# KamilSJaron/smudgeplot

Measured on NVIDIA H100. Metric: k-mers/sec scanned (hetmers) at 1/2/4/8 H100; bit-exact .smu vs ref C, higher is better.
Workload: dtype u64

## Files before the change

### include/hetmers_b200.h

```cpp
#ifndef HETMERS_B200_H
#define HETMERS_B200_H

#include <stdint.h>

#ifdef __cplusplus
extern "C" {
#endif

#define HM_SMAX        1000
#define HM_FMAX         500
#define HM_PLOT_W      (HM_FMAX+1)
#define HM_PLOT_CELLS  ((HM_SMAX+1)*(HM_FMAX+1))
#define HM_MAX_KMER      64
#define HM_MAX_SHARDS    16
#define HM_FILTER_MIN_BITS 22
#define HM_FILTER_MAX_BITS 37

#define HM_OK            0
#define HM_EINVAL       -1
#define HM_ECUDA        -2
#define HM_ENOMEM       -3
#define HM_EIO          -4
#define HM_EFORMAT      -5
#define HM_EUNSUPPORTED -6
// ... 51 lines not shown
                       unsigned long long *d_count, const hm_shards *shards, void *stream);

#define HM_SYMM_MIN_KMER 2

typedef struct hm_symm_layout
  { int64_t bytes;
    int64_t off_header;
    int64_t off_bloom;
    int64_t seg_words;
    int64_t off_cand_key, off_cand_lo, off_cand_meta;
    int64_t cand_cap;
    int64_t range;
    int64_t off_runs, runs_cap;
    int32_t n_seg, pad;
  } hm_symm_layout;

typedef struct hm_symm_shards
  { int32_t  n_seg, self;
    int64_t  off[HM_MAX_SHARDS+1];
    uint64_t first_key[HM_MAX_SHARDS];
  } hm_symm_shards;

#define HM_SYMM_ASYMMETRIC 1
#define HM_SYMM_OVERFLOW   2

int  hm_symm_plan(int64_t n, int64_t range, int kmer, int n_seg, hm_symm_layout *out);
void hm_symm_seeds(uint64_t seed[2]);
int  hm_k_symm_fingerprint(const uint64_t *d_keys, const uint64_t *d_keys_lo, const uint16_t *d_cnt,
                           int64_t i0, int64_t i1, int kmer, const uint64_t seed[2],
                           uint64_t *d_acc, void *stream);
int  hm_k_symm_runscan(const uint64_t *d_keys, const uint64_t *d_keys_lo, const uint16_t *d_cnt, int64_t n,
                       const void *d_bucket, int bits, int idx64, int kmer, int64_t lo, int64_t hi,
                       void *d_work, const hm_symm_layout *layout, const hm_symm_shards *shards, void *stream);
int  hm_k_symm_runs(const uint64_t *d_keys, const uint64_t *d_keys_lo, const uint16_t *d_cnt, int64_t n,
                    const void *d_bucket, int bits, int idx64, int kmer, int64_t lo, int64_t hi,
                    void *d_work, const hm_symm_layout *layout, const hm_symm_shards *shards, void *stream);
int  hm_k_symm_resolve(const uint64_t *d_keys, const uint64_t *d_keys_lo, const uint16_t *d_cnt, int64_t n,
                       const void *d_bucket, int bits, int idx64, int kmer,
                       void *d_work, const hm_symm_layout *layout, const hm_symm_shards *shards,
                       unsigned long long *d_plot, void *stream);
int  hm_k_symm_extract(const uint64_t *d_keys, const uint64_t *d_keys_lo, const uint16_t *d_cnt, int64_t n,
                       const void *d_bucket, int bits, int idx64, int kmer,
                       void *d_work, const hm_symm_layout *layout, const hm_symm_shards *shards,
                       const uint16_t *d_pixmap, int64_t c0, int64_t c1, hm_pair_rec *d_out, int64_t cap,
                       unsigned long long *d_count, void *stream);
int  hm_symm_status(const void *d_work, const hm_symm_layout *layout, uint64_t *n_cand, uint64_t *status,
                    void *stream);
int  hm_symm_align_cut(const uint64_t *d_keys, int64_t n, int kmer, int64_t cut, int64_t *out);

int hm_dev_alloc(int64_t bytes, void **dptr);
int hm_dev_free(void *dptr);
int hm_ipc_export(void *dptr, unsigned char handle[64]);
int hm_ipc_open(const unsigned char handle[64], void **dptr);
int hm_ipc_close(void *dptr);
int hm_p2p_native_atomics(int dev_a, int dev_b);

int hm_k_min_count(const uint16_t *d_cnt, int64_t frst, int64_t last, int *d_min, void *stream);

int hm_k_find_keys(const uint64_t *d_keys, const uint64_t *d_keys_lo, int64_t n,
                   const void *d_bucket, int bits, int idx64,
                   const uint64_t *d_query, const uint64_t *d_query_lo, int64_t nq,
                   int64_t *d_pos, void *stream);

int hm_pick_bucket_bits(int64_t n);


// ... 211 lines not shown
```

### smudgeplot_b200/_lib.py

```python
from __future__ import annotations

import ctypes as C
import os

HERE = os.path.dirname(os.path.abspath(__file__))
LIB_PATH = os.environ.get("HETMERS_LIB") or os.path.join(HERE, "lib", "libhetmers_b200.so")
BIN_PATH = os.path.join(HERE, "bin", "hetmers")

SMAX, FMAX = 1000, 500
PLOT_W = FMAX + 1
PLOT_CELLS = (SMAX + 1) * (FMAX + 1)

ABI_SYMBOLS = [
    "hm_last_error", "hm_abi_version", "hm_device_count", "hm_device_info",
    "hm_k_unpack_records", "hm_k_build_bucket_index", "hm_k_pass1_degree", "hm_k_pass2_plot",
    "hm_k_min_count", "hm_k_find_keys", "hm_pick_bucket_bits", "hm_k_pass2_extract", "hm_scan_extract", "hm_pass2_scratch_bytes",
    "hm_k_build_filter", "hm_filter_words", "hm_pick_filter_bits",
    "hm_dev_alloc", "hm_dev_free", "hm_ipc_export", "hm_ipc_open", "hm_ipc_close", "hm_p2p_native_atomics",
    "hm_scan_create", "hm_prewarm", "hm_set_io_threads", "hm_scan_destroy", "hm_scan_examine", "hm_scan_condition", "hm_scan_run", "hm_hetmers_host",
    "hm_scan_run_path", "hm_scan_is_symmetric", "hm_symm_plan", "hm_symm_seeds", "hm_k_symm_fingerprint", "hm_k_symm_runscan", "hm_k_symm_runs", "hm_k_symm_resolve",
    "hm_k_symm_extract",
    "hm_symm_status", "hm_symm_align_cut",
    "hm_scan_download", "hm_set_device_budget", "hm_stream_plan", "hm_stream_plan_shards", "hm_scan_residency", "hm_table_open", "hm_table_close", "hm_table_view", "hm_write_smu",
    "hm_rank_scan_create", "hm_rank_scan_destroy", "hm_rank_scan_cuts", "hm_rank_scan_pass1", "hm_rank_scan_bloom",
    "hm_rank_scan_prepare", "hm_rank_scan_slices", "hm_rank_scan_route", "hm_rank_scan_answer", "hm_rank_scan_settle",
    "hm_rank_scan_result", "hm_rank_scan_residency",
    "hm_rank_scan_extract_prepare", "hm_rank_scan_extract_slices", "hm_rank_scan_extract_route",
    "hm_rank_scan_extract_settle", "hm_rank_scan_extract_result", "hm_sort_pair_records",
    "hm_condition_range_bytes", "hm_condition_plan", "hm_scan_condition_files",
    "hm_table_write_open", "hm_table_write_buckets", "hm_table_write_append", "hm_table_write_close",
    "hm_table_write_abort", "hm_table_write_place", "hm_table_write_at", "hm_table_write_seal",
    "hm_set_condition_gpus",
    "hm_k_cond_hist", "hm_k_shard_route_count", "hm_k_shard_route_scatter", "hm_k_shard_settle_bytes",
    "hm_k_shard_settle", "hm_shard_condition_bytes",
    "hm_k_shard_route_count_window", "hm_k_shard_route_scatter_window", "hm_k_cond_pack", "hm_rank_condition_bytes",
    "hm_rank_condition_cut",
    "hm_rank_scan_extract_records", "hm_k_pairs_hist", "hm_k_pairs_route_count", "hm_k_pairs_route_scatter",
    "hm_pairs_sort_scratch_bytes", "hm_k_pairs_sort", "hm_k_pairs_label_bounds", "hm_k_pairs_format", "hm_pairs_bytes",
    "hm_scan_write_pairs", "hm_scan_pairs_hist", "hm_pair_windows",
]


class HostTable(C.Structure):
    _fields_ = [("kmer", C.c_int32), ("ibyte", C.c_int32), ("nparts", C.c_int32), ("minval", C.c_int32),
                ("nels", C.c_int64), ("index", C.POINTER(C.c_int64)), ("part_nels", C.POINTER(C.c_int64)),
                ("part_rec", C.POINTER(C.c_void_p)), ("part_fd", C.POINTER(C.c_int32)),
                ("part_fd_off", C.POINTER(C.c_int64))]


MAX_SHARDS = 16


class Shards(C.Structure):
# ... 90 lines not shown
    if not os.path.exists(LIB_PATH):
        raise ImportError(f"{LIB_PATH} is missing: run `make lib` (or __graft_entry__.build()); "
                          "the hetmers path has no CPU / PyTorch fallback")
    L = C.CDLL(LIB_PATH)
    vp, i32, i64 = C.c_void_p, C.c_int, C.c_int64
    L.hm_last_error.restype = C.c_char_p
    L.hm_device_info.argtypes = [i32, C.c_char_p, i32, C.POINTER(i32), C.POINTER(i64)]
    L.hm_k_unpack_records.argtypes = [vp, i64, i64, vp, i32, i32, vp, vp, vp, vp]
    L.hm_k_build_bucket_index.argtypes = [vp, i64, i32, vp, i32, vp]
    L.hm_k_pass1_degree.argtypes = [vp, vp, vp, i64, vp, i32, i32, vp, i32, i32, i64, i64, vp, vp, C.POINTER(Shards), vp]
    L.hm_dev_alloc.argtypes = [i64, C.POINTER(vp)]
    L.hm_dev_free.argtypes = [vp]
    L.hm_ipc_export.argtypes = [vp, C.c_char_p]
    L.hm_ipc_open.argtypes = [C.c_char_p, C.POINTER(vp)]
    L.hm_ipc_close.argtypes = [vp]
    L.hm_p2p_native_atomics.argtypes = [i32, i32]
    L.hm_k_build_filter.argtypes = [vp, i64, i32, vp, vp]
    L.hm_filter_words.argtypes = [i32]
    L.hm_filter_words.restype = i64
    L.hm_pick_filter_bits.argtypes = [i64]
    L.hm_k_pass2_plot.argtypes = [vp, vp, vp, i32, i64, i64, vp, C.POINTER(Shards), vp]
    L.hm_k_pass2_extract.argtypes = [vp, vp, vp, vp, vp, i32, i64, i64, vp, vp, i64, vp, C.POINTER(Shards), vp]
    L.hm_k_min_count.argtypes = [vp, i64, i64, vp, vp]
    L.hm_k_find_keys.argtypes = [vp, vp, i64, vp, i32, i32, vp, vp, i64, vp, vp]
    L.hm_pick_bucket_bits.argtypes = [i64]
    L.hm_pass2_scratch_bytes.argtypes = [i64, i32]
    L.hm_pass2_scratch_bytes.restype = i64
    L.hm_symm_plan.argtypes = [i64, i64, i32, i32, C.POINTER(SymmLayout)]
    L.hm_symm_seeds.argtypes = [C.POINTER(C.c_uint64)]
    L.hm_symm_seeds.restype = None
    L.hm_k_symm_fingerprint.argtypes = [vp, vp, vp, i64, i64, i32, C.POINTER(C.c_uint64), vp, vp]
    L.hm_k_symm_runscan.argtypes = [vp, vp, vp, i64, vp, i32, i32, i32, i64, i64, vp, C.POINTER(SymmLayout),
                                    C.POINTER(SymmShards), vp]
    L.hm_k_symm_runs.argtypes = [vp, vp, vp, i64, vp, i32, i32, i32, i64, i64, vp, C.POINTER(SymmLayout),
                                 C.POINTER(SymmShards), vp]
    L.hm_k_symm_resolve.argtypes = [vp, vp, vp, i64, vp, i32, i32, i32, vp, C.POINTER(SymmLayout),
                                    C.POINTER(SymmShards), vp, vp]
    L.hm_k_symm_extract.argtypes = [vp, vp, vp, i64, vp, i32, i32, i32, vp, C.POINTER(SymmLayout),
                                    C.POINTER(SymmShards), vp, i64, i64, vp, i64, vp, vp]
    L.hm_symm_status.argtypes = [vp, C.POINTER(SymmLayout), C.POINTER(C.c_uint64), C.POINTER(C.c_uint64), vp]
    L.hm_symm_align_cut.argtypes = [vp, i64, i32, i64, C.POINTER(i64)]
    L.hm_scan_create.argtypes = [C.POINTER(HostTable), C.POINTER(i32), i32, C.POINTER(vp)]
    L.hm_scan_destroy.argtypes = [vp]
    L.hm_scan_destroy.restype = None
    L.hm_scan_examine.argtypes = [vp, i32, C.POINTER(i32), C.POINTER(i32)]
    L.hm_scan_condition.argtypes = [vp, i32, i32, i32, C.POINTER(i64)]
    L.hm_scan_run.argtypes = [vp, vp, C.POINTER(ScanStats)]
    L.hm_scan_run_path.argtypes = [vp, i32, vp, C.POINTER(ScanStats)]
    L.hm_scan_is_symmetric.argtypes = [vp]
    L.hm_scan_extract.argtypes = [vp, vp, C.POINTER(C.POINTER(PairRec)), C.POINTER(i64)]
    L.hm_hetmers_host.argtypes = [C.POINTER(HostTable), C.POINTER(i32), i32, vp, C.POINTER(ScanStats)]
    L.hm_scan_download.argtypes = [vp, vp, vp, vp, vp]
    L.hm_set_device_budget.argtypes = [i64]
    L.hm_set_device_budget.restype = None
    L.hm_stream_plan.argtypes = [i64, i32, i32, i64, C.POINTER(StreamLayout)]
    L.hm_stream_plan_shards.argtypes = [i64, i32, i32, i64, i32, C.POINTER(StreamLayout)]
    L.hm_scan_residency.argtypes = [vp, C.POINTER(i64), C.POINTER(i64)]
    u64p, i64p = C.POINTER(C.c_uint64), C.POINTER(i64)
    L.hm_rank_scan_create.argtypes = [C.POINTER(HostTable), i32, i32, i32, u64p, C.POINTER(vp)]
    L.hm_rank_scan_destroy.argtypes = [vp]
    L.hm_rank_scan_destroy.restype = None
    L.hm_rank_scan_cuts.argtypes = [vp, i64p, u64p]
    L.hm_rank_scan_pass1.argtypes = [vp, u64p]
    L.hm_rank_scan_bloom.argtypes = [vp, C.POINTER(vp), i64p]
    L.hm_rank_scan_prepare.argtypes = [vp, i32, i64p, i64p]
    L.hm_rank_scan_slices.argtypes = [vp, i64, i64p, C.POINTER(vp), C.POINTER(vp), C.POINTER(vp), C.POINTER(vp)]
# ... 68 lines not shown
```

### smudgeplot_b200/csrc/hm_symm.cu

```cuda
#include <cuda_runtime.h>
#include <stdint.h>
#include <stdio.h>
#include <stdlib.h>
#include <string.h>

#include "hetmers_b200.h"
#include "hm_internal.h"
#include "hm_device.cuh"

#define RS_THREADS 256
#define RS_EPT     8
#define RS_TILE    (RS_THREADS*RS_EPT)
#define RS_HALO    64
#define RS_WIN     (RS_TILE+2*RS_HALO)
#define RS_SCANCAP RS_HALO
#define RS_RUNCAP  (RS_HALO+1)
#define RS_LONGRUN 32
#ifndef RS_MINBLOCKS
#define RS_MINBLOCKS 6
#endif
#ifndef RS_STAGE
#define RS_STAGE   384
#endif

#define SY_STATUS_ASYMMETRIC 1ull
#define SY_STATUS_OVERFLOW   2ull

#define SY_HDR_CAND   0
#define SY_HDR_STATUS 1
#define SY_HDR_RUNS   2
#define SY_HDR_S      3
#define SY_HDR_PEND   4
#define SY_HDR_QUERY  5

struct SymmView
  { unsigned long long *cand_n;
    unsigned long long *status;
    uint32_t *bloom;
    uint32_t  seg_words;
    int       n_seg, self;
    uint64_t  first_key[HM_MAX_SHARDS];
    uint64_t *cand_key, *cand_lo, *cand_meta;
    unsigned long long cand_cap;
    unsigned long long *runs_n;
    uint64_t *runs;
    unsigned long long runs_cap;
    uint64_t *s_key, *s_lo;
    unsigned long long s_cap;
    const hm_stream_sview *sviews;
    uint64_t *pend, *pend_key, *pend_lo;
    uint64_t *q_key, *q_lo, *q_tag;
    unsigned long long pend_cap, q_cap;
  };

template <int KW>
__device__ __forceinline__ void bloom_slot(const SymmView &W, int seg, int kmer, uint64_t hi, uint64_t lo,
// ... 204 lines not shown
static int l2_persist(void)
{ const char *e = getenv("HETMERS_L2_PERSIST");
  return (e == NULL || strcmp(e,"0") != 0);
}

static SymmView make_view(void *d_work, const hm_symm_layout *L, const hm_symm_shards *sh)
{ SymmView W;
  uint8_t *b = (uint8_t *) d_work;
  memset(&W,0,sizeof(W));
  W.cand_n    = (unsigned long long *) (b + L->off_header) + SY_HDR_CAND;
  W.status    = W.cand_n + SY_HDR_STATUS;
  W.bloom     = (uint32_t *) (b + L->off_bloom);
  W.seg_words = (uint32_t) L->seg_words;
  W.n_seg     = L->n_seg;
  W.self      = 0;
  if (sh != NULL && sh->n_seg > 1)
    { W.self = sh->self;
      for (int r = 0; r < sh->n_seg; r++) W.first_key[r] = sh->first_key[r];
    }
  W.cand_key  = (uint64_t *) (b + L->off_cand_key);
  W.cand_lo   = (uint64_t *) (b + L->off_cand_lo);
  W.cand_meta = (uint64_t *) (b + L->off_cand_meta);
  W.cand_cap  = (unsigned long long) L->cand_cap;
  W.runs_n    = W.cand_n + SY_HDR_RUNS;
  W.runs      = (uint64_t *) (b + L->off_runs);
  W.runs_cap  = (unsigned long long) L->runs_cap;
  return W;
}


template <int KW> struct RsSmem
  { uint64_t *key, *klo;
    uint16_t *cnt;
    uint64_t *ckey, *clo, *cmeta;
    uint16_t *t1;
    uint16_t *t2r;
  };

__device__ __forceinline__ uint64_t pack_meta(int cx, int cy, int pos, int yb)
{ return (uint64_t) cx | ((uint64_t) cy << 16) | ((uint64_t) pos << 32) | ((uint64_t) yb << 40); }

#ifdef RS_PROBE
__device__ int rs_probe_mode;
#define RS_PROBE_IS(m) (rs_probe_mode == (m))
#else
#define RS_PROBE_IS(m) false
#endif

template <int KW>
__device__ __forceinline__ void stage_candidates(const RsSmem<KW> &S, unsigned *s_nc, const SymmView &W,
                                                 bool emit, uint64_t x, uint64_t xl, uint64_t meta,
                                                 int lane, unsigned lt)
{ const unsigned bal = __ballot_sync(0xffffffffu,emit);
  if (bal == 0 || RS_PROBE_IS(4))
    return;
  unsigned base = 0;
  if (lane == 0)
    base = atomicAdd(s_nc,(unsigned) __popc(bal));
  base = __shfl_sync(0xffffffffu,base,0);
  const unsigned at = base + __popc(bal & lt);
  const bool     over = emit && (at >= RS_STAGE);
  if (emit && !over)
    { S.ckey[at] = x;
      if (KW == 2) S.clo[at] = xl;
      S.cmeta[at] = meta;
    }
  if (base + __popc(bal) <= RS_STAGE)
    return;
  const unsigned ob = __ballot_sync(0xffffffffu,over);
  unsigned long long g0 = 0;
  if (lane == 0)
    g0 = atomicAdd(W.cand_n,(unsigned long long) __popc(ob));
  g0 = __shfl_sync(0xffffffffu,g0,0) + (unsigned long long) __popc(ob & lt);
  if (over)
    { if (g0 < W.cand_cap)
        { W.cand_key[g0] = x;
          if (KW == 2) W.cand_lo[g0] = xl;
          W.cand_meta[g0] = meta;
        }
      else
        atomicOr(W.status,SY_STATUS_OVERFLOW);
    }
}

template <int KW>
__device__ __forceinline__ void s_push(const SymmView &W, uint64_t x, uint64_t xl)
{ const unsigned m = __activemask();
  const int      lane = threadIdx.x & 31, lead = __ffs(m)-1;
  unsigned long long at = 0;
  if (lane == lead)
    at = atomicAdd(W.cand_n + SY_HDR_S,(unsigned long long) __popc(m));
  at = __shfl_sync(m,at,lead) + (unsigned long long) __popc(m & ((1u << lane)-1));
  if (at < W.s_cap)
    { W.s_key[at] = x;
      if (KW == 2) W.s_lo[at] = xl;
    }
  else
    atomicOr(W.status,SY_STATUS_OVERFLOW);
}

template <int KW, bool SL>
__device__ __forceinline__ void bloom_insert(const SymmView &W, int kmer, uint64_t x, uint64_t xl)
{ uint64_t *word, mask;
  bloom_slot<KW>(W,W.self,kmer,x,xl,word,mask);
  if (!RS_PROBE_IS(3) || mask == (uint64_t) (uintptr_t) word)
    red_or64(word,mask);
  if (SL)
    s_push<KW>(W,x,xl);
}

#define RS_FLUSH ((RS_STAGE+RS_THREADS-1)/RS_THREADS)
struct RsFlush { uint64_t key[RS_FLUSH], lo[RS_FLUSH], meta[RS_FLUSH]; };

template <int KW>
__device__ __forceinline__ void flush_reserve(const RsSmem<KW> &S, unsigned long long *s_cb,
                                              unsigned long long *s_rb, const SymmView &W,
                                              unsigned nc, unsigned nr, RsFlush &F)
{ if (threadIdx.x == 0)
    { if (nc > 0) *s_cb = atomicAdd(W.cand_n,(unsigned long long) nc);
      if (nr > 0) *s_rb = atomicAdd(W.runs_n,(unsigned long long) nr);
    }
#pragma unroll
  for (int j = 0; j < RS_FLUSH; j++)
    { const unsigned i = threadIdx.x + j*RS_THREADS;
      if (i < nc)
        { F.key[j] = S.ckey[i];
          if (KW == 2) F.lo[j] = S.clo[i];
          F.meta[j] = S.cmeta[i];
        }
    }
}

template <int KW>
__device__ __forceinline__ void flush_store(const RsSmem<KW> &S, unsigned long long cb, unsigned long long rb,
                                            const SymmView &W, unsigned nc, unsigned nr, int64_t T0,
                                            const RsFlush &F)
{
#pragma unroll
  for (int j = 0; j < RS_FLUSH; j++)
    { const unsigned i = threadIdx.x + j*RS_THREADS;
      if (i < nc)
        { if (cb+i < W.cand_cap)
            { W.cand_key[cb+i] = F.key[j];
              if (KW == 2) W.cand_lo[cb+i] = F.lo[j];
              W.cand_meta[cb+i] = F.meta[j];
            }
          else
            atomicOr(W.status,SY_STATUS_OVERFLOW);
        }
    }
  for (unsigned i = threadIdx.x; i < nr; i += RS_THREADS)
    if (rb+i < W.runs_cap)
      W.runs[rb+i] = (uint64_t) (T0 + ((int) S.t2r[i] - RS_HALO));
    else
      atomicOr(W.status,SY_STATUS_OVERFLOW);
}

template <typename IdxT, int KW, bool SL>
__global__ void __launch_bounds__(256)
runs_kernel(const uint64_t *__restrict__ keys, const uint64_t *__restrict__ keys_lo,
            const uint16_t *__restrict__ cnt, int64_t n, const IdxT *__restrict__ bucket, int bshift,
            int kmer, int64_t lo, int64_t hi, const SymmView W)
// ... 65 lines not shown
                          if (KW == 2) W.cand_lo[base] = xl;
                          W.cand_meta[base] = meta;
                        }
                      else
                        atomicOr(W.status,SY_STATUS_OVERFLOW);
                    }
                }
            }
        }
    }
}

template <int KW> struct RunSfx    { typedef uint64_t T; };
template <>       struct RunSfx<1> { typedef uint32_t T; };

template <int KW>
__device__ __forceinline__ typename RunSfx<KW>::T run_sfx(uint64_t hi, uint64_t lo, int Pr)
{ if constexpr (KW == 1)
    return (uint32_t) ((hi << 2*Pr) >> 32);
  else
    return (hi << (2*Pr-32) << 32) | (lo >> (64-2*Pr));
}

template <typename T>
__device__ __forceinline__ bool one_base_in_run(T d, int Pr, int &pos)
{ const T u = (d | (d >> 1)) & (T) HM_M5;
  if constexpr (sizeof(T) == 4) pos = Pr + (__clz((int) d) >> 1);
  else                          pos = Pr + (__clzll((long long) d) >> 1);
  return (u & (u-1)) == 0;
}

template <int KW, bool SL, int LMAX>
__device__ __forceinline__ bool settle_members(const RsSmem<KW> &S, const SymmView &W, int kmer, int Pr, int pup,
                                               int h, int L, int a, bool in, bool own, int lane,
                                               uint64_t &x, uint64_t &xl, uint64_t &meta)
{ int Hx = 0, Ux = 0, part = 0, ppos = 0, cx = 0;
  if (in)
    { x  = S.key[h+a];
      xl = KW == 2 ? S.klo[h+a] : 0;
      cx = S.cnt[h+a];
      auto mate = [&](int b)
        { int pos;
          if (b < L && b != a && one_base_in_run(run_sfx<KW>(x ^ S.key[h+b],KW == 2 ? xl ^ S.klo[h+b] : 0,Pr),Pr,pos) &&
              cx + (int) S.cnt[h+b] <= HM_SMAX)
            { Hx += 1;
              if (pos >= pup) Ux += 1;
              part = b; ppos = pos;
            }
        };
      if constexpr (LMAX > 0)
        {
#pragma unroll
          for (int b = 0; b < LMAX; b++)
            mate(b);
        }
      else
        for (int b = 0; b < L; b++)
          mate(b);
      if (own && Ux > 0)
        bloom_insert<KW,SL>(W,kmer,x,xl);
    }
  const int pl = lane + part - a;
  int       Hy = __shfl_sync(0xffffffffu,Hx,pl & 31);
  if (!in || !own || Hx != 1 || part < a)
    return false;
  const uint64_t y = S.key[h+part], yl = KW == 2 ? S.klo[h+part] : 0;
  const int      cy = S.cnt[h+part];
  if (pl > 31)
    { Hy = 0;
      for (int b = 0; b < L; b++)
        { int pos;
          if (b != part && one_base_in_run(run_sfx<KW>(y ^ S.key[h+b],KW == 2 ? yl ^ S.klo[h+b] : 0,Pr),Pr,pos) &&
              cy + (int) S.cnt[h+b] <= HM_SMAX)
            Hy += 1;
        }
    }
  if (Hy != 1)
    return false;
  meta = pack_meta(cx,cy,ppos,base_at<KW>(y,yl,ppos));
  return true;
}

#ifdef RS_PROBE
#define RS_PHASES 8
#define RS_COLS   (RS_PHASES+3)
#define RS_PROBE_SLOTS 1024
__device__ unsigned long long rs_probe_cycles[RS_PROBE_SLOTS*RS_COLS];
#define RS_PROBE_TILE(b)  (rs_probe_mode == 2 ? (b) % 64 : (b))
#define RS_PROBE_START    __shared__ long long rs_t0, rs_t1; \
                          long long rs_t = clock64(); unsigned long long rs_acc[RS_PHASES] = {0, 0, 0, 0, 0, 0, 0, 0}; \
                          if (threadIdx.x == 0) rs_t0 = rs_t;
#define RS_PROBE_MARK(ph) { const long long t_ = clock64(); rs_acc[ph] += (unsigned long long) (t_ - rs_t); rs_t = t_; }
#define RS_PROBE_LANDED() if (threadIdx.x == 0) rs_t1 = clock64();
#define RS_PROBE_ALLDONE  const long long rs_t2 = clock64();
#define RS_PROBE_ROW      (rs_probe_cycles + (blockIdx.x % RS_PROBE_SLOTS)*RS_COLS)
#define RS_PROBE_FLUSH()  { if (lane == 0) _Pragma("unroll") for (int p_ = 0; p_ < RS_PHASES; p_++) \
                              atomicAdd(RS_PROBE_ROW + p_,rs_acc[p_]); }
#define RS_PROBE_LIFE()   { const long long t3_ = clock64(); \
                            if (threadIdx.x == 0) { atomicAdd(RS_PROBE_ROW + RS_PHASES,  (unsigned long long) (rs_t1 - rs_t0)); \
                                             atomicAdd(RS_PROBE_ROW + RS_PHASES+1,(unsigned long long) (rs_t2 - rs_t1)); \
                                             atomicAdd(RS_PROBE_ROW + RS_PHASES+2,(unsigned long long) (t3_ - rs_t2)); } }
#define RS_PROBE_LOADONLY() if (rs_probe_mode == 1) { RS_PROBE_FLUSH(); return; }
#define RS_PROBE_NOTAIL()   if (rs_probe_mode == 6) { RS_PROBE_FLUSH(); return; }

extern "C" int hm_probe_runscan(int mode, unsigned long long *cycles)
{ static unsigned long long rows[RS_PROBE_SLOTS*RS_COLS];
  cudaError_t e = cudaDeviceSynchronize();
  if (e == cudaSuccess && cycles != NULL)
    { e = cudaMemcpyFromSymbol(rows,rs_probe_cycles,sizeof(rows));
      for (int p = 0; p < RS_COLS; p++)
        { cycles[p] = 0;
          for (int r = 0; r < RS_PROBE_SLOTS; r++)
            cycles[p] += rows[r*RS_COLS+p];
        }
    }
  memset(rows,0,sizeof(rows));
  if (e == cudaSuccess)
    e = cudaMemcpyToSymbol(rs_probe_cycles,rows,sizeof(rows));
  if (e == cudaSuccess)
    e = cudaMemcpyToSymbol(rs_probe_mode,&mode,sizeof(mode));
  return e == cudaSuccess ? HM_OK : hm_cuda_fail(e,"hm_probe_runscan");
}
#else
#define RS_PROBE_TILE(b)  (b)
#define RS_PROBE_START
#define RS_PROBE_MARK(ph)
#define RS_PROBE_LANDED()
#define RS_PROBE_ALLDONE
#define RS_PROBE_FLUSH()
#define RS_PROBE_LIFE()
#define RS_PROBE_LOADONLY()
#define RS_PROBE_NOTAIL()
#endif

template <typename IdxT, int KW, bool SL>
__global__ void __launch_bounds__(RS_THREADS,RS_MINBLOCKS)
runscan_kernel(const uint64_t *__restrict__ keys, const uint64_t *__restrict__ keys_lo,
               const uint16_t *__restrict__ cnt, int64_t n, const IdxT *__restrict__ bucket, int bshift,
               int kmer, int64_t lo, int64_t hi, int64_t tile0, int use_tma, const SymmView W)
{ extern __shared__ __align__(128) uint8_t smem[];
  __shared__ __align__(8) uint64_t s_bar;
  __shared__ unsigned s_nc, s_nr;
  __shared__ unsigned long long s_base[2];
  RsSmem<KW> S;
  S.key   = (uint64_t *) smem;
  S.klo   = S.key + (KW == 2 ? RS_WIN : 0);
  S.ckey  = S.key + KW*RS_WIN;
  S.clo   = S.ckey + (KW == 2 ? RS_STAGE : 0);
  S.cmeta = S.ckey + KW*RS_STAGE;
  S.cnt   = (uint16_t *) (S.cmeta + RS_STAGE);
  S.t1    = S.cnt + RS_WIN;
  S.t2r   = S.t1 + RS_TILE/2;

  const int      Pr   = kmer >> 1;
  const int      pup  = kmer - Pr;
  const int      psh  = 64-2*Pr;
  const uint64_t pmask = ~(uint64_t) 0 << psh;
  const unsigned FULL = 0xffffffffu;
  const int      lane = threadIdx.x & 31;
  const int      warp = threadIdx.x >> 5;
  const unsigned lt   = (1u << lane) - 1;
  RS_PROBE_START

  const int64_t T0 = (tile0 + RS_PROBE_TILE(blockIdx.x)) * RS_TILE;
  const int64_t ws = T0 - RS_HALO;
  const int64_t e0 = ws > 0 ? ws : 0;
  const int64_t e1 = T0+RS_TILE+RS_HALO < n ? T0+RS_TILE+RS_HALO : n;
  const int     v0 = (int) (e0-ws), v1 = (int) (e1-ws);

  const int m   = v1-v0;
  const int mt  = use_tma ? (m & ~7) : 0;
  if (threadIdx.x == 0)
    { s_nc = 0; s_nr = 0;
      if (mt > 0)
        { mbar_init(&s_bar,1);
          fence_proxy_async_smem();
        }
    }
  __syncthreads();
  if (threadIdx.x == 0 && mt > 0)
    { mbar_arrive_expect_tx(&s_bar,(unsigned) (mt*(8*KW+2)));
      bulk_copy_g2s(S.key+v0,keys+e0,(unsigned) (8*mt),&s_bar);
      if (KW == 2)
// ... 59 lines not shown
        if (s0+32 > a1)   act &= (a1-s0 <= 0)  ? 0u : (0xffffffffu >> (s0+32-a1));
        const unsigned more = (em1 & E) | (E & ep1) | (em1 & em2);
        m2 = (E & ~em1 & ~ep1) & act;
        m3 = more & act & ~em1;
      }
    const int c2 = __popc(m2), c3 = __popc(m3);
    int pre2 = c2, pre3 = c3;
#pragma unroll
    for (int o = 1; o <= RS_EPT; o <<= 1)
      { int v2 = __shfl_up_sync(FULL,pre2,o), v3 = __shfl_up_sync(FULL,pre3,o);
        if (lane >= o) { pre2 += v2; pre3 += v3; }
      }
    n1 = __shfl_sync(FULL,pre2,RS_EPT);
    n3 = __shfl_sync(FULL,pre3,RS_EPT);
    int at = pre2-c2;
    while (m2 != 0)
      { my1[at++] = (uint16_t) (wd*32 + __ffs(m2)-1);
        m2 &= m2-1;
      }
    at = n1 + pre3-c3;
    while (m3 != 0)
      { my1[at++] = (uint16_t) (wd*32 + __ffs(m3)-1);
        m3 &= m3-1;
      }
  }
  __syncwarp();
  if (RS_PROBE_IS(5))
    n3 = 0;
  RS_PROBE_MARK(2)

  for (int i0 = 0; i0 < n1; i0 += 32)
    { const int i = i0+lane;
      bool     emit = false;
      uint64_t x = 0, xl = 0, meta = 0;
      if (i < n1)
        { const int w = my1[i];
          x = S.key[w];
          const uint64_t y = S.key[w+1];
          uint64_t yl = 0;
          if (KW == 2) { xl = S.klo[w]; yl = S.klo[w+1]; }
          const int cx = S.cnt[w], cy = S.cnt[w+1];
          int pos;
          if (one_base_in_run(run_sfx<KW>(x ^ y,xl ^ yl,Pr),Pr,pos) && cx+cy <= HM_SMAX)
            { emit = true;
              meta = pack_meta(cx,cy,pos,base_at<KW>(y,yl,pos));
              if (pos >= pup)
                { bloom_insert<KW,SL>(W,kmer,x,xl);
                  bloom_insert<KW,SL>(W,kmer,y,yl);
                }
            }
        }
      stage_candidates<KW>(S,&s_nc,W,emit,x,xl,meta,lane,lt);
    }
  RS_PROBE_MARK(3)

  const int b1 = hi-T0 < RS_TILE+RS_HALO ? RS_HALO + (int) (hi-T0) : RS_WIN;
  for (int i0 = 0; i0 < n3; i0 += 32)
    { const int i = i0+lane;
      const int h = i < n3 ? my1[n1+i] : 0;
      int       L = 0;
      {
        const int      t  = (h >> 5) - (wd0-1);
        const unsigned w0 = __shfl_sync(FULL,eqw,t & 31), w1 = __shfl_sync(FULL,eqw,(t+1) & 31);
        const unsigned up = __funnelshift_r(w0,w1,h & 31);
        if (i < n3)
          L = (~up != 0) ? __ffs((int) ~up) : 33;
      }
      const int Ls = L <= 8 ? L : 0;
      int inc = Ls;
#pragma unroll
      for (int o = 1; o < 32; o <<= 1)
        { const int v = __shfl_up_sync(FULL,inc,o);
          if (lane >= o) inc += v;
        }
      const int M = __shfl_sync(FULL,inc,31);
      for (int t0 = 0; t0 < M; t0 += 32)
        { const int t = t0+lane;
          int r = 0;
#pragma unroll
          for (int s = 16; s > 0; s >>= 1)
            if (__shfl_sync(FULL,inc,r+s-1) <= t) r += s;
          const int hr = __shfl_sync(FULL,h,r), Lr = __shfl_sync(FULL,Ls,r);
          const int a  = t - (__shfl_sync(FULL,inc,r) - Lr);
          bool     emit = false;
          uint64_t x = 0, xl = 0, meta = 0;
          emit = settle_members<KW,SL,8>(S,W,kmer,Pr,pup,hr,Lr,a,t < M,hr+a < b1,lane,x,xl,meta);
          stage_candidates<KW>(S,&s_nc,W,emit,x,xl,meta,lane,lt);
        }
      unsigned lb = __ballot_sync(FULL,L > 8);
      while (lb != 0)
        { const int src = __ffs(lb)-1;
          lb &= lb-1;
          const int hh = __shfl_sync(FULL,h,src);
          int       LL = __shfl_sync(FULL,L,src);
          if (LL > 32)
            { const uint64_t xh = S.key[hh];
              while (LL <= RS_RUNCAP)
                { const int      t = hh+LL+lane;
                  const unsigned sb = __ballot_sync(FULL,t < RS_WIN && ((S.key[t] ^ xh) & pmask) == 0);
                  if (sb != FULL) { LL += __ffs(~sb)-1; break; }
                  LL += 32;
                }
            }
          if (LL > RS_RUNCAP || hh+LL >= RS_WIN)
            { if (lane == 0)
                S.t2r[atomicAdd(&s_nr,1u)] = (uint16_t) hh;
              continue;
            }
          for (int a0 = 0; a0 < LL; a0 += 32)
            { const int a = a0+lane;
              bool     emit = false;
              uint64_t x = 0, xl = 0, meta = 0;
              emit = settle_members<KW,SL,0>(S,W,kmer,Pr,pup,hh,LL,a,a < LL,hh+a < b1,lane,x,xl,meta);
              stage_candidates<KW>(S,&s_nc,W,emit,x,xl,meta,lane,lt);
            }
        }
    }
  RS_PROBE_MARK(4)
  RS_PROBE_NOTAIL()

  __syncthreads();
  RS_PROBE_MARK(5)
  RS_PROBE_ALLDONE
  if (RS_PROBE_IS(4))
    { RS_PROBE_FLUSH() return; }
  const unsigned nc = s_nc < RS_STAGE ? s_nc : RS_STAGE, nr = s_nr;
  if (nc == 0 && nr == 0)
    { RS_PROBE_MARK(6) RS_PROBE_LIFE() RS_PROBE_FLUSH() return; }
  RsFlush F;
  flush_reserve<KW>(S,&s_base[0],&s_base[1],W,nc,nr,F);
  __syncthreads();
  RS_PROBE_MARK(6)
  flush_store<KW>(S,s_base[0],s_base[1],W,nc,nr,T0,F);
  RS_PROBE_MARK(7)
  RS_PROBE_LIFE()
  RS_PROBE_FLUSH()
}

template <typename IdxT, int KW, bool SL>
__global__ void __launch_bounds__(RS_THREADS,RS_MINBLOCKS)
runscan_dense_kernel(const uint64_t *__restrict__ keys, const uint64_t *__restrict__ keys_lo,
                     const uint16_t *__restrict__ cnt, int64_t n, int kmer, int64_t lo, int64_t hi,
                     int64_t tile0, int use_tma, const SymmView W)
{ extern __shared__ __align__(128) uint8_t smem[];
  __shared__ __align__(8) uint64_t s_bar;
  __shared__ unsigned s_nc, s_nl;
  __shared__ unsigned long long s_base[2];
  __shared__ unsigned s_eq[RS_WIN/32+1];
  RsSmem<KW> S;
  S.key   = (uint64_t *) smem;
  S.klo   = S.key + (KW == 2 ? RS_WIN : 0);
  S.ckey  = S.key + KW*RS_WIN;
  S.clo   = S.ckey + (KW == 2 ? RS_STAGE : 0);
  S.cmeta = S.ckey + KW*RS_STAGE;
  S.cnt   = (uint16_t *) (S.cmeta + RS_STAGE);
  S.t1    = S.cnt + RS_WIN;
  S.t2r   = S.t1 + RS_WIN;
  uint16_t *s_part = S.t2r + RS_TILE/8;
  unsigned *hu = (unsigned *) (s_part + RS_WIN);
  uint32_t *rem = hu + RS_WIN/2;

  const int      Pr   = kmer >> 1, pup = kmer - Pr, psh = 64-2*Pr;
  const uint64_t pmask = ~(uint64_t) 0 << psh;
  const unsigned FULL = 0xffffffffu;
  const int      lane = threadIdx.x & 31;
  const int      warp = threadIdx.x >> 5;
  const unsigned lt   = (1u << lane) - 1;

  const int64_t T0 = (tile0 + blockIdx.x) * RS_TILE;
  const int64_t ws = T0 - RS_HALO;
  const int64_t e0 = ws > 0 ? ws : 0;
  const int64_t e1 = T0+RS_TILE+RS_HALO < n ? T0+RS_TILE+RS_HALO : n;
  const int     v0 = (int) (e0-ws), v1 = (int) (e1-ws);

  const int m   = v1-v0;
  const int mt  = use_tma ? (m & ~7) : 0;
  if (threadIdx.x == 0)
    { s_nc = 0; s_nl = 0;
      if (mt > 0)
        { mbar_init(&s_bar,1);
          fence_proxy_async_smem();
        }
    }
  for (int j = threadIdx.x; j < RS_WIN/2; j += RS_THREADS)
    hu[j] = 0;
  __syncthreads();
  if (threadIdx.x == 0 && mt > 0)
    { mbar_arrive_expect_tx(&s_bar,(unsigned) (mt*(8*KW+2)));
// ... 70 lines not shown
        { const uint32_t rx = rem[i];
          for (int j = i+1; j <= i+fwd; j++)
            { const uint32_t d = rx ^ rem[j];
              const uint32_t u = (d | (d>>1)) & 0x55555555u;
              if ((u & (u-1)) == 0 && cx + (int) S.cnt[j] <= HM_SMAX)
                { const int      pos = Pr + (__clz((int) d) >> 1);
                  const unsigned inc = 1u | (pos >= pup ? 0x100u : 0u);
                  atomicAdd(hu + (i>>1), inc << (16*(i&1)));
                  atomicAdd(hu + (j>>1), inc << (16*(j&1)));
                  s_part[i] = (uint16_t) j;
                  s_part[j] = (uint16_t) i;
                }
            }
        }
      else
        { const uint64_t x = S.key[i], xl = KW == 2 ? S.klo[i] : 0;
          for (int j = i+1; j <= i+fwd; j++)
            { int pos;
              if (one_base_apart<KW>(x,xl,S.key[j],KW == 2 ? S.klo[j] : 0,pos) && cx + (int) S.cnt[j] <= HM_SMAX)
                { const unsigned inc = 1u | (pos >= pup ? 0x100u : 0u);
                  atomicAdd(hu + (i>>1), inc << (16*(i&1)));
                  atomicAdd(hu + (j>>1), inc << (16*(j&1)));
                  s_part[i] = (uint16_t) j;
                  s_part[j] = (uint16_t) i;
                }
            }
        }
    }
  __syncthreads();

  for (int i0 = RS_HALO + (threadIdx.x & ~31); i0 < RS_HALO+RS_TILE; i0 += RS_THREADS)
    { const int i = i0+lane;
      bool     emit = false;
      uint64_t x = 0, xl = 0, meta = 0;
      if (i >= a0 && i < a1 && S.t1[i] != 0xffff)
        { const unsigned c = (hu[i>>1] >> (16*(i&1))) & 0xffffu;
          const int H = (int) (c & 0xff), U = (int) (c >> 8);
          if (H > 0)
            { x = S.key[i];
              if (KW == 2) xl = S.klo[i];
              if (U > 0)
                bloom_insert<KW,SL>(W,kmer,x,xl);
              const int j = s_part[i];
              if (H == 1 && j > i && ((hu[j>>1] >> (16*(j&1))) & 0xffu) == 1)
                { const uint64_t y = S.key[j], yl = KW == 2 ? S.klo[j] : 0;
                  int pos;
                  one_base_apart<KW>(x,xl,y,yl,pos);
                  emit = true;
                  meta = pack_meta(S.cnt[i],S.cnt[j],pos,base_at<KW>(y,yl,pos));
                }
            }
        }
      stage_candidates<KW>(S,&s_nc,W,emit,x,xl,meta,lane,lt);
    }

  __syncthreads();
  const unsigned nc = s_nc < RS_STAGE ? s_nc : RS_STAGE, nr = s_nl;
  if (nc == 0 && nr == 0)
    return;
  RsFlush F;
  flush_reserve<KW>(S,&s_base[0],&s_base[1],W,nc,nr,F);
  __syncthreads();
  flush_store<KW>(S,s_base[0],s_base[1],W,nc,nr,T0,F);
}

template <typename I, int K> struct Inst { typedef I IdxT; static constexpr int KW = K; };

template <class F>
static cudaError_t dispatch(int kmer, int idx64, F f)
{ if (kmer <= 32)
    return idx64 ? f(Inst<uint64_t,1>()) : f(Inst<uint32_t,1>());
  return idx64 ? f(Inst<uint64_t,2>()) : f(Inst<uint32_t,2>());
}

template <typename IdxT, int KW, bool SL = false>
static cudaError_t launch_runscan(const uint64_t *keys, const uint64_t *keys_lo, const uint16_t *cnt, int64_t n,
                                  const void *bucket, int bits, int kmer, int64_t lo, int64_t hi,
                                  const SymmView &W, cudaStream_t st)
{ static int configured[64] = {0};
  int dev = 0;
  cudaGetDevice(&dev);
  int64_t tile0 = lo/RS_TILE, tile1 = (hi+RS_TILE-1)/RS_TILE;
  int     tma   = ((((uintptr_t) keys) | ((uintptr_t) cnt) | ((uintptr_t) (keys_lo ? keys_lo : keys))) & 15) == 0;
  const int   Pr  = kmer >> 1;
  double      lam = (2*Pr >= 62) ? 0.0 : (double) n / (double) ((uint64_t) 1 << (2*Pr));
  bool        dense = (lam > 0.6);
  const char *force = getenv("HETMERS_RUNSCAN");
  if (force != NULL && strcmp(force,"dense") == 0)  dense = true;
  if (force != NULL && strcmp(force,"sparse") == 0) dense = false;
  cudaError_t e;
  if (dense)
    { size_t smem = (size_t) RS_WIN*(8*KW+2) + (size_t) RS_STAGE*8*(KW+1) +
                    2*(size_t) (RS_WIN+RS_TILE/8+RS_WIN) + 4*(size_t) (RS_WIN/2+RS_WIN);
      if (smem > 48*1024 && (dev >= 64 || !(configured[dev] & 2)))
        { e = cudaFuncSetAttribute(runscan_dense_kernel<IdxT,KW,SL>,cudaFuncAttributeMaxDynamicSharedMemorySize,(int) smem);
          if (e != cudaSuccess) return e;
          if (dev < 64) configured[dev] |= 2;
        }
      runscan_dense_kernel<IdxT,KW,SL><<<(unsigned) (tile1-tile0),RS_THREADS,smem,st>>>
          (keys,keys_lo,cnt,n,kmer,lo,hi,tile0,tma,W);
    }
  else
    { size_t smem = (size_t) RS_WIN*(8*KW+2) + (size_t) RS_STAGE*8*(KW+1) +
                    2*(size_t) (RS_TILE/2+RS_TILE/2);
      if (smem > 48*1024 && (dev >= 64 || !(configured[dev] & 1)))
        { e = cudaFuncSetAttribute(runscan_kernel<IdxT,KW,SL>,cudaFuncAttributeMaxDynamicSharedMemorySize,(int) smem);
          if (e != cudaSuccess) return e;
          if (dev < 64) configured[dev] |= 1;
        }
      runscan_kernel<IdxT,KW,SL><<<(unsigned) (tile1-tile0),RS_THREADS,smem,st>>>
          (keys,keys_lo,cnt,n,(const IdxT *) bucket,64-bits,kmer,lo,hi,tile0,tma,W);
    }
  return cudaGetLastError();
}

template <typename IdxT, int KW, bool SL = false>
static cudaError_t launch_runs(const uint64_t *keys, const uint64_t *keys_lo, const uint16_t *cnt, int64_t n,
                               const void *bucket, int bits, int kmer, int64_t lo, int64_t hi,
                               const SymmView &W, cudaStream_t st)
{
  int dev = 0, sms = 132;
  cudaGetDevice(&dev);
  cudaDeviceGetAttribute(&sms,cudaDevAttrMultiProcessorCount,dev);
  int64_t want = ((hi-lo)/64+255)/256;
  int     grid = (int) (want < sms*8 ? (want > 0 ? want : 1) : sms*8);
  runs_kernel<IdxT,KW,SL><<<grid,256,0,st>>>(keys,keys_lo,cnt,n,(const IdxT *) bucket,64-bits,kmer,lo,hi,W);
  return cudaGetLastError();
}

extern "C" int hm_k_symm_runscan(const uint64_t *d_keys, const uint64_t *d_keys_lo, const uint16_t *d_cnt, int64_t n,
                                 const void *d_bucket, int bits, int idx64, int kmer, int64_t lo, int64_t hi,
                                 void *d_work, const hm_symm_layout *layout, const hm_symm_shards *shards,
                                 void *stream)
{ if (kmer < HM_SYMM_MIN_KMER || kmer > HM_MAX_KMER)
    return hm_set_error(HM_EUNSUPPORTED,"symmetric scan needs %d <= k <= %d (k=%d)",HM_SYMM_MIN_KMER,HM_MAX_KMER,kmer);
  if (lo < 0 || hi > n || lo > hi || bits < 1 || bits > 30 || d_work == NULL || layout == NULL)
    return hm_set_error(HM_EINVAL,"symm_runscan: bad range [%lld,%lld) of %lld or bits %d",
                        (long long) lo,(long long) hi,(long long) n,bits);
  if ((kmer > 32) != (d_keys_lo != NULL))
    return hm_set_error(HM_EINVAL,"symm_runscan: second key word array %s for k=%d",
                        d_keys_lo ? "given" : "missing",kmer);
  if ((shards != NULL && shards->n_seg > 1) != (layout->n_seg > 1) ||
      (shards != NULL && shards->n_seg > 1 && (shards->n_seg != layout->n_seg || shards->self < 0 ||
                                               shards->self >= shards->n_seg)))
    return hm_set_error(HM_EINVAL,"symm_runscan: shard table does not match the work-area layout");
  cudaStream_t st = (cudaStream_t) stream;
  SymmView W = make_view(d_work,layout,shards);
  HM_CUDA(cudaMemsetAsync(W.cand_n,0,256,st));
  HM_CUDA(cudaMemsetAsync(W.bloom + (size_t) W.self*W.seg_words,0,sizeof(uint32_t)*(size_t) W.seg_words,st));
  if (l2_persist())
    bloom_window(st,W.bloom,sizeof(uint32_t)*(size_t) W.seg_words*(size_t) W.n_seg,1);
  if (hi == lo)
    return HM_OK;
  cudaError_t e = dispatch(kmer,idx64,[&](auto I)
    { return launch_runscan<typename decltype(I)::IdxT,decltype(I)::KW>(d_keys,d_keys_lo,d_cnt,n,d_bucket,bits,kmer,
                                                                       lo,hi,W,st); });
  if (e != cudaSuccess)
    return hm_cuda_fail(e,"runscan_kernel");
  return HM_OK;
}

extern "C" int hm_k_symm_runs(const uint64_t *d_keys, const uint64_t *d_keys_lo, const uint16_t *d_cnt, int64_t n,
                              const void *d_bucket, int bits, int idx64, int kmer, int64_t lo, int64_t hi,
                              void *d_work, const hm_symm_layout *layout, const hm_symm_shards *shards,
                              void *stream)
{ if (kmer < HM_SYMM_MIN_KMER || kmer > HM_MAX_KMER || d_work == NULL || layout == NULL ||
      (kmer > 32) != (d_keys_lo != NULL) || lo < 0 || hi > n || lo > hi)
    return hm_set_error(HM_EINVAL,"symm_runs: bad arguments");
  if (hi == lo)
    return HM_OK;
  cudaStream_t st = (cudaStream_t) stream;
  SymmView W = make_view(d_work,layout,shards);
  cudaError_t e = dispatch(kmer,idx64,[&](auto I)
    { return launch_runs<typename decltype(I)::IdxT,decltype(I)::KW>(d_keys,d_keys_lo,d_cnt,n,d_bucket,bits,kmer,
                                                                    lo,hi,W,st); });
  if (e != cudaSuccess)
    return hm_cuda_fail(e,"runs_kernel");
  return HM_OK;
}


#define RV_TS   192
#define RV_TM   96
#define RV_TROW 97
#define RV_THREADS 1024
#ifndef RV_ILP
#define RV_ILP 2
#endif
#define RV_QCAP  (32*(RV_ILP+1))
#define RV_PROBE 4
#define RV_HA    (1ull << 48)
#define RV_HB    (1ull << 49)
// ... 1023 lines not shown
```

Before: 135.7 billion.

## Pack staged runscan candidates into 32-bit window indices to raise occupancy

```diff
diff --git a/include/hetmers_b200.h b/include/hetmers_b200.h
--- a/include/hetmers_b200.h
+++ b/include/hetmers_b200.h
@@ -107,6 +107,7 @@
 int  hm_k_symm_runscan(const uint64_t *d_keys, const uint64_t *d_keys_lo, const uint16_t *d_cnt, int64_t n,
                        const void *d_bucket, int bits, int idx64, int kmer, int64_t lo, int64_t hi,
                        void *d_work, const hm_symm_layout *layout, const hm_symm_shards *shards, void *stream);
+int  hm_runscan_occupancy(int kmer, int idx64, int *blocks);
 int  hm_k_symm_runs(const uint64_t *d_keys, const uint64_t *d_keys_lo, const uint16_t *d_cnt, int64_t n,
                     const void *d_bucket, int bits, int idx64, int kmer, int64_t lo, int64_t hi,
                     void *d_work, const hm_symm_layout *layout, const hm_symm_shards *shards, void *stream);
diff --git a/smudgeplot_b200/_lib.py b/smudgeplot_b200/_lib.py
--- a/smudgeplot_b200/_lib.py
+++ b/smudgeplot_b200/_lib.py
@@ -18,7 +18,7 @@
     "hm_k_build_filter", "hm_filter_words", "hm_pick_filter_bits",
     "hm_dev_alloc", "hm_dev_free", "hm_ipc_export", "hm_ipc_open", "hm_ipc_close", "hm_p2p_native_atomics",
     "hm_scan_create", "hm_prewarm", "hm_set_io_threads", "hm_scan_destroy", "hm_scan_examine", "hm_scan_condition", "hm_scan_run", "hm_hetmers_host",
-    "hm_scan_run_path", "hm_scan_is_symmetric", "hm_symm_plan", "hm_symm_seeds", "hm_k_symm_fingerprint", "hm_k_symm_runscan", "hm_k_symm_runs", "hm_k_symm_resolve",
+    "hm_scan_run_path", "hm_scan_is_symmetric", "hm_symm_plan", "hm_symm_seeds", "hm_k_symm_fingerprint", "hm_k_symm_runscan", "hm_runscan_occupancy", "hm_k_symm_runs", "hm_k_symm_resolve",
     "hm_k_symm_extract",
     "hm_symm_status", "hm_symm_align_cut",
     "hm_scan_download", "hm_set_device_budget", "hm_stream_plan", "hm_stream_plan_shards", "hm_scan_residency", "hm_table_open", "hm_table_close", "hm_table_view", "hm_write_smu",
@@ -175,6 +175,7 @@
     L.hm_k_symm_fingerprint.argtypes = [vp, vp, vp, i64, i64, i32, C.POINTER(C.c_uint64), vp, vp]
     L.hm_k_symm_runscan.argtypes = [vp, vp, vp, i64, vp, i32, i32, i32, i64, i64, vp, C.POINTER(SymmLayout),
                                     C.POINTER(SymmShards), vp]
+    L.hm_runscan_occupancy.argtypes = [i32, i32, C.POINTER(i32)]
     L.hm_k_symm_runs.argtypes = [vp, vp, vp, i64, vp, i32, i32, i32, i64, i64, vp, C.POINTER(SymmLayout),
                                  C.POINTER(SymmShards), vp]
     L.hm_k_symm_resolve.argtypes = [vp, vp, vp, i64, vp, i32, i32, i32, vp, C.POINTER(SymmLayout),
diff --git a/smudgeplot_b200/csrc/hm_symm.cu b/smudgeplot_b200/csrc/hm_symm.cu
--- a/smudgeplot_b200/csrc/hm_symm.cu
+++ b/smudgeplot_b200/csrc/hm_symm.cu
@@ -19,9 +19,18 @@
 #ifndef RS_MINBLOCKS
 #define RS_MINBLOCKS 6
 #endif
+#define RS_MINBLOCKS_K32 8
 #ifndef RS_STAGE
 #define RS_STAGE   384
 #endif
+
+static constexpr size_t runscan_smem(int KW)
+  { return (size_t) RS_WIN*(8*KW+2) + 4*(size_t) RS_STAGE + 2*(size_t) (RS_TILE/2+RS_TILE/2); }
+static constexpr size_t runscan_dense_smem(int KW)
+  { return (size_t) RS_WIN*(8*KW+2) + 4*(size_t) RS_STAGE + 2*(size_t) (RS_WIN+RS_TILE/8+RS_WIN) +
+           4*(size_t) (RS_WIN/2+RS_WIN); }
+#define RS_SMEM_K32 (runscan_smem(1) + 128 + 1024)
+static_assert(RS_MINBLOCKS_K32*RS_SMEM_K32 <= 228*1024, "eight k <= 32 runscan_kernel CTAs fit in an SM's 228 KB");
 
 #define SY_STATUS_ASYMMETRIC 1ull
 #define SY_STATUS_OVERFLOW   2ull
@@ -292,13 +301,28 @@
 template <int KW> struct RsSmem
   { uint64_t *key, *klo;
     uint16_t *cnt;
-    uint64_t *ckey, *clo, *cmeta;
+    uint32_t *cand;
     uint16_t *t1;
     uint16_t *t2r;
   };
 
 __device__ __forceinline__ uint64_t pack_meta(int cx, int cy, int pos, int yb)
 { return (uint64_t) cx | ((uint64_t) cy << 16) | ((uint64_t) pos << 32) | ((uint64_t) yb << 40); }
+
+static_assert(RS_WIN <= (1 << 12), "a window slot takes 12 bits of a staged candidate");
+static_assert(RS_RUNCAP-1 < (1 << 7) && RS_LONGRUN-1 < (1 << 7), "a partner lies at most 127 slots after x");
+static_assert(HM_MAX_KMER <= (1 << 6), "a position takes 6 bits of a staged candidate");
+
+__device__ __forceinline__ uint32_t stage_word(int xs, int ys, int pos, int yb)
+{ return (uint32_t) xs | ((uint32_t) (ys-xs) << 12) | ((uint32_t) pos << 19) | ((uint32_t) yb << 25); }
+
+template <int KW>
+__device__ __forceinline__ void unstage(const RsSmem<KW> &S, uint32_t c, uint64_t &x, uint64_t &xl, uint64_t &meta)
+{ const int xs = (int) (c & 0xfffu), ys = xs + (int) ((c >> 12) & 0x7fu);
+  x  = S.key[xs];
+  xl = KW == 2 ? S.klo[xs] : 0;
+  meta = pack_meta(S.cnt[xs],S.cnt[ys],(int) ((c >> 19) & 0x3fu),(int) (c >> 25));
+}
 
 #ifdef RS_PROBE
 __device__ int rs_probe_mode;
@@ -309,8 +333,7 @@
 
 template <int KW>
 __device__ __forceinline__ void stage_candidates(const RsSmem<KW> &S, unsigned *s_nc, const SymmView &W,
-                                                 bool emit, uint64_t x, uint64_t xl, uint64_t meta,
-                                                 int lane, unsigned lt)
+                                                 bool emit, uint32_t c, int lane, unsigned lt)
 { const unsigned bal = __ballot_sync(0xffffffffu,emit);
   if (bal == 0 || RS_PROBE_IS(4))
     return;
@@ -321,10 +344,7 @@
   const unsigned at = base + __popc(bal & lt);
   const bool     over = emit && (at >= RS_STAGE);
   if (emit && !over)
-    { S.ckey[at] = x;
-      if (KW == 2) S.clo[at] = xl;
-      S.cmeta[at] = meta;
-    }
+    S.cand[at] = c;
   if (base + __popc(bal) <= RS_STAGE)
     return;
   const unsigned ob = __ballot_sync(0xffffffffu,over);
@@ -334,7 +354,9 @@
   g0 = __shfl_sync(0xffffffffu,g0,0) + (unsigned long long) __popc(ob & lt);
   if (over)
     { if (g0 < W.cand_cap)
-        { W.cand_key[g0] = x;
+        { uint64_t x, xl, meta;
+          unstage<KW>(S,c,x,xl,meta);
+          W.cand_key[g0] = x;
           if (KW == 2) W.cand_lo[g0] = xl;
           W.cand_meta[g0] = meta;
         }
@@ -384,10 +406,7 @@
   for (int j = 0; j < RS_FLUSH; j++)
     { const unsigned i = threadIdx.x + j*RS_THREADS;
       if (i < nc)
-        { F.key[j] = S.ckey[i];
-          if (KW == 2) F.lo[j] = S.clo[i];
-          F.meta[j] = S.cmeta[i];
-        }
+        unstage<KW>(S,S.cand[i],F.key[j],F.lo[j],F.meta[j]);
     }
 }
 
@@ -519,9 +538,9 @@
 
 template <int KW, bool SL, int LMAX>
 __device__ __forceinline__ bool settle_members(const RsSmem<KW> &S, const SymmView &W, int kmer, int Pr, int pup,
-                                               int h, int L, int a, bool in, bool own, int lane,
-                                               uint64_t &x, uint64_t &xl, uint64_t &meta)
+                                               int h, int L, int a, bool in, bool own, int lane, uint32_t &c)
 { int Hx = 0, Ux = 0, part = 0, ppos = 0, cx = 0;
+  uint64_t x = 0, xl = 0;
   if (in)
     { x  = S.key[h+a];
       xl = KW == 2 ? S.klo[h+a] : 0;
@@ -564,7 +583,7 @@
     }
   if (Hy != 1)
     return false;
-  meta = pack_meta(cx,cy,ppos,base_at<KW>(y,yl,ppos));
+  c = stage_word(h+a,h+part,ppos,base_at<KW>(y,yl,ppos));
   return true;
 }
 
@@ -621,7 +640,7 @@
 #endif
 
 template <typename IdxT, int KW, bool SL>
-__global__ void __launch_bounds__(RS_THREADS,RS_MINBLOCKS)
+__global__ void __launch_bounds__(RS_THREADS,KW == 1 && !SL ? RS_MINBLOCKS_K32 : RS_MINBLOCKS)
 runscan_kernel(const uint64_t *__restrict__ keys, const uint64_t *__restrict__ keys_lo,
                const uint16_t *__restrict__ cnt, int64_t n, const IdxT *__restrict__ bucket, int bshift,
                int kmer, int64_t lo, int64_t hi, int64_t tile0, int use_tma, const SymmView W)
@@ -632,10 +651,8 @@
   RsSmem<KW> S;
   S.key   = (uint64_t *) smem;
   S.klo   = S.key + (KW == 2 ? RS_WIN : 0);
-  S.ckey  = S.key + KW*RS_WIN;
-  S.clo   = S.ckey + (KW == 2 ? RS_STAGE : 0);
-  S.cmeta = S.ckey + KW*RS_STAGE;
-  S.cnt   = (uint16_t *) (S.cmeta + RS_STAGE);
+  S.cand  = (uint32_t *) (S.key + KW*RS_WIN);
+  S.cnt   = (uint16_t *) (S.cand + RS_STAGE);
   S.t1    = S.cnt + RS_WIN;
   S.t2r   = S.t1 + RS_TILE/2;
 
@@ -761,25 +778,24 @@
   for (int i0 = 0; i0 < n1; i0 += 32)
     { const int i = i0+lane;
       bool     emit = false;
-      uint64_t x = 0, xl = 0, meta = 0;
+      uint32_t c = 0;
       if (i < n1)
         { const int w = my1[i];
-          x = S.key[w];
-          const uint64_t y = S.key[w+1];
-          uint64_t yl = 0;
+          const uint64_t x = S.key[w], y = S.key[w+1];
+          uint64_t xl = 0, yl = 0;
           if (KW == 2) { xl = S.klo[w]; yl = S.klo[w+1]; }
           const int cx = S.cnt[w], cy = S.cnt[w+1];
           int pos;
           if (one_base_in_run(run_sfx<KW>(x ^ y,xl ^ yl,Pr),Pr,pos) && cx+cy <= HM_SMAX)
             { emit = true;
-              meta = pack_meta(cx,cy,pos,base_at<KW>(y,yl,pos));
+              c = stage_word(w,w+1,pos,base_at<KW>(y,yl,pos));
               if (pos >= pup)
                 { bloom_insert<KW,SL>(W,kmer,x,xl);
                   bloom_insert<KW,SL>(W,kmer,y,yl);
                 }
             }
         }
-      stage_candidates<KW>(S,&s_nc,W,emit,x,xl,meta,lane,lt);
+      stage_candidates<KW>(S,&s_nc,W,emit,c,lane,lt);
     }
   RS_PROBE_MARK(3)
 
@@ -802,7 +818,8 @@
         { const int v = __shfl_up_sync(FULL,inc,o);
           if (lane >= o) inc += v;
         }
-      const int M = __shfl_sync(FULL,inc,31);
+      const int  M = __shfl_sync(FULL,inc,31);
+      const bool upto4 = __all_sync(FULL,Ls <= 4);
       for (int t0 = 0; t0 < M; t0 += 32)
         { const int t = t0+lane;
           int r = 0;
@@ -811,10 +828,10 @@
             if (__shfl_sync(FULL,inc,r+s-1) <= t) r += s;
           const int hr = __shfl_sync(FULL,h,r), Lr = __shfl_sync(FULL,Ls,r);
           const int a  = t - (__shfl_sync(FULL,inc,r) - Lr);
-          bool     emit = false;
-          uint64_t x = 0, xl = 0, meta = 0;
-          emit = settle_members<KW,SL,8>(S,W,kmer,Pr,pup,hr,Lr,a,t < M,hr+a < b1,lane,x,xl,meta);
-          stage_candidates<KW>(S,&s_nc,W,emit,x,xl,meta,lane,lt);
+          uint32_t c = 0;
+          const bool emit = upto4 ? settle_members<KW,SL,4>(S,W,kmer,Pr,pup,hr,Lr,a,t < M,hr+a < b1,lane,c)
+                                  : settle_members<KW,SL,8>(S,W,kmer,Pr,pup,hr,Lr,a,t < M,hr+a < b1,lane,c);
+          stage_candidates<KW>(S,&s_nc,W,emit,c,lane,lt);
         }
       unsigned lb = __ballot_sync(FULL,L > 8);
       while (lb != 0)
@@ -838,10 +855,9 @@
             }
           for (int a0 = 0; a0 < LL; a0 += 32)
             { const int a = a0+lane;
-              bool     emit = false;
-              uint64_t x = 0, xl = 0, meta = 0;
-              emit = settle_members<KW,SL,0>(S,W,kmer,Pr,pup,hh,LL,a,a < LL,hh+a < b1,lane,x,xl,meta);
-              stage_candidates<KW>(S,&s_nc,W,emit,x,xl,meta,lane,lt);
+              uint32_t c = 0;
+              const bool emit = settle_members<KW,SL,0>(S,W,kmer,Pr,pup,hh,LL,a,a < LL,hh+a < b1,lane,c);
+              stage_candidates<KW>(S,&s_nc,W,emit,c,lane,lt);
             }
         }
     }
@@ -879,10 +895,8 @@
   RsSmem<KW> S;
   S.key   = (uint64_t *) smem;
   S.klo   = S.key + (KW == 2 ? RS_WIN : 0);
-  S.ckey  = S.key + KW*RS_WIN;
-  S.clo   = S.ckey + (KW == 2 ? RS_STAGE : 0);
-  S.cmeta = S.ckey + KW*RS_STAGE;
-  S.cnt   = (uint16_t *) (S.cmeta + RS_STAGE);
+  S.cand  = (uint32_t *) (S.key + KW*RS_WIN);
+  S.cnt   = (uint16_t *) (S.cand + RS_STAGE);
   S.t1    = S.cnt + RS_WIN;
   S.t2r   = S.t1 + RS_WIN;
   uint16_t *s_part = S.t2r + RS_TILE/8;
@@ -1019,13 +1033,12 @@
   for (int i0 = RS_HALO + (threadIdx.x & ~31); i0 < RS_HALO+RS_TILE; i0 += RS_THREADS)
     { const int i = i0+lane;
       bool     emit = false;
-      uint64_t x = 0, xl = 0, meta = 0;
+      uint32_t cw = 0;
       if (i >= a0 && i < a1 && S.t1[i] != 0xffff)
         { const unsigned c = (hu[i>>1] >> (16*(i&1))) & 0xffffu;
           const int H = (int) (c & 0xff), U = (int) (c >> 8);
           if (H > 0)
-            { x = S.key[i];
-              if (KW == 2) xl = S.klo[i];
+            { const uint64_t x = S.key[i], xl = KW == 2 ? S.klo[i] : 0;
               if (U > 0)
                 bloom_insert<KW,SL>(W,kmer,x,xl);
               const int j = s_part[i];
@@ -1034,11 +1047,11 @@
                   int pos;
                   one_base_apart<KW>(x,xl,y,yl,pos);
                   emit = true;
-                  meta = pack_meta(S.cnt[i],S.cnt[j],pos,base_at<KW>(y,yl,pos));
+                  cw = stage_word(i,j,pos,base_at<KW>(y,yl,pos));
                 }
             }
         }
-      stage_candidates<KW>(S,&s_nc,W,emit,x,xl,meta,lane,lt);
+      stage_candidates<KW>(S,&s_nc,W,emit,cw,lane,lt);
     }
 
   __syncthreads();
@@ -1058,6 +1071,16 @@
 { if (kmer <= 32)
     return idx64 ? f(Inst<uint64_t,1>()) : f(Inst<uint32_t,1>());
   return idx64 ? f(Inst<uint64_t,2>()) : f(Inst<uint32_t,2>());
+}
+
+template <typename IdxT, int KW, bool SL>
+static cudaError_t runscan_attributes(void)
+{ cudaError_t e = cudaFuncSetAttribute(runscan_kernel<IdxT,KW,SL>,cudaFuncAttributeMaxDynamicSharedMemorySize,
+                                       (int) runscan_smem(KW));
+  if (e == cudaSuccess)
+    e = cudaFuncSetAttribute(runscan_kernel<IdxT,KW,SL>,cudaFuncAttributePreferredSharedMemoryCarveout,
+                             (int) cudaSharedmemCarveoutMaxShared);
+  return e;
 }
 
 template <typename IdxT, int KW, bool SL = false>
@@ -1077,8 +1100,7 @@
   if (force != NULL && strcmp(force,"sparse") == 0) dense = false;
   cudaError_t e;
   if (dense)
-    { size_t smem = (size_t) RS_WIN*(8*KW+2) + (size_t) RS_STAGE*8*(KW+1) +
-                    2*(size_t) (RS_WIN+RS_TILE/8+RS_WIN) + 4*(size_t) (RS_WIN/2+RS_WIN);
+    { const size_t smem = runscan_dense_smem(KW);
       if (smem > 48*1024 && (dev >= 64 || !(configured[dev] & 2)))
         { e = cudaFuncSetAttribute(runscan_dense_kernel<IdxT,KW,SL>,cudaFuncAttributeMaxDynamicSharedMemorySize,(int) smem);
           if (e != cudaSuccess) return e;
@@ -1088,14 +1110,12 @@
           (keys,keys_lo,cnt,n,kmer,lo,hi,tile0,tma,W);
     }
   else
-    { size_t smem = (size_t) RS_WIN*(8*KW+2) + (size_t) RS_STAGE*8*(KW+1) +
-                    2*(size_t) (RS_TILE/2+RS_TILE/2);
-      if (smem > 48*1024 && (dev >= 64 || !(configured[dev] & 1)))
-        { e = cudaFuncSetAttribute(runscan_kernel<IdxT,KW,SL>,cudaFuncAttributeMaxDynamicSharedMemorySize,(int) smem);
+    { if (dev >= 64 || !(configured[dev] & 1))
+        { e = runscan_attributes<IdxT,KW,SL>();
           if (e != cudaSuccess) return e;
           if (dev < 64) configured[dev] |= 1;
         }
-      runscan_kernel<IdxT,KW,SL><<<(unsigned) (tile1-tile0),RS_THREADS,smem,st>>>
+      runscan_kernel<IdxT,KW,SL><<<(unsigned) (tile1-tile0),RS_THREADS,runscan_smem(KW),st>>>
           (keys,keys_lo,cnt,n,(const IdxT *) bucket,64-bits,kmer,lo,hi,tile0,tma,W);
     }
   return cudaGetLastError();
@@ -1145,6 +1165,20 @@
   if (e != cudaSuccess)
     return hm_cuda_fail(e,"runscan_kernel");
   return HM_OK;
+}
+
+extern "C" int hm_runscan_occupancy(int kmer, int idx64, int *blocks)
+{ if (kmer < HM_SYMM_MIN_KMER || kmer > HM_MAX_KMER || blocks == NULL)
+    return hm_set_error(HM_EINVAL,"runscan_occupancy: k=%d",kmer);
+  cudaError_t e = dispatch(kmer,idx64,[&](auto I)
+    { typedef typename decltype(I)::IdxT IdxT;
+      constexpr int KW = decltype(I)::KW;
+      cudaError_t r = runscan_attributes<IdxT,KW,false>();
+      if (r == cudaSuccess)
+        r = cudaOccupancyMaxActiveBlocksPerMultiprocessor(blocks,runscan_kernel<IdxT,KW,false>,RS_THREADS,
+                                                          runscan_smem(KW));
+      return r; });
+  return e == cudaSuccess ? HM_OK : hm_cuda_fail(e,"runscan_occupancy");
 }
 
 extern "C" int hm_k_symm_runs(const uint64_t *d_keys, const uint64_t *d_keys_lo, const uint16_t *d_cnt, int64_t n,
```

Measured after the change: 135.4 billion, median of 6. Within noise of the previous version (-0.3%).
